# HIITMetagenomics/dsm-framework

Hardware: AMD Instinct MI355X
Metric: enumerated substrings/sec (Emax=2.0) (higher is better)
Workload: dtype u32

## Files before the change

dsm-framework_amd/csrc/engine.hip:

```cpp
#include <sched.h>

#include <algorithm>
#include <atomic>
#include <chrono>
#include <cmath>
#include <condition_variable>
#include <cstdlib>
#include <cstring>
#include <deque>
#include <map>
#include <functional>
#include <memory>
#include <mutex>
#include <sstream>
#include <thread>
#include <type_traits>

#include "common.h"
#include "scan.h"
#include "setorder.h"
#include "stream_parse.h"
#include "lfstep.h"
#include "entropy_tables.h"
#include "textemit.h"
#include "engine_api.h"
#include "emit_runs.h"

namespace dsm {

__device__ __forceinline__ u64 wave_sum_u64(u64 v) {
#pragma unroll
    for (int d = 32; d >= 1; d >>= 1) v += __shfl_xor(v, d, 64);
    return v;
}


struct Kids {
    const u64* plane;
    const u32* cum;
};
__device__ __forceinline__ u32 kid_mask(const Kids& k, u32 v) {
    const u64* p = k.plane + (size_t)(v >> 6) * 4;
    const u32 s = v & 63;
    return (u32)((p[0] >> s) & 1) | ((u32)((p[1] >> s) & 1) << 1) | ((u32)((p[2] >> s) & 1) << 2) | ((u32)((p[3] >> s) & 1) << 3);
}
__device__ __forceinline__ u32 kid_index(const Kids& k, u32 v, u32 c) {
    const size_t e = (size_t)(v >> 6) * 4 + c;
    return k.cum[e] + (u32)__popcll(k.plane[e] & ((1ull << (v & 63)) - 1));
}

struct KidWave {
    u64 p[4];
    u32 c[4];
};
__device__ __forceinline__ void kid_wave(const Kids& k, u32 w, KidWave& o) {
#pragma unroll
    for (int c = 0; c < 4; ++c) { o.p[c] = k.plane[(size_t)w * 4 + c]; o.c[c] = k.cum[(size_t)w * 4 + c]; }
}
__device__ __forceinline__ u32 bits_below_lane(u64 p) {
    return __builtin_amdgcn_mbcnt_hi((u32)(p >> 32), __builtin_amdgcn_mbcnt_lo((u32)p, 0u));
}

constexpr u32 NUM_XCD = 8;
__device__ __forceinline__ u32 xcd_block() {
    const u32 b = blockIdx.x, G = gridDim.x;
    const u32 x = b % NUM_XCD, i = b / NUM_XCD, per = G / NUM_XCD, rem = G % NUM_XCD;
    return x * per + (x < rem ? x : rem) + i;
}

constexpr int NPT = 4;
static inline dim3 grid_npt(u64 n) { return dim3((unsigned)((n + 256ull * NPT - 1) / (256ull * NPT))); }


static inline void timeline(const char* what, const char* arg = "") {
    static const bool on = getenv("DSM_TIMELINE") != nullptr;
    if (!on) return;
    static const auto t0 = std::chrono::steady_clock::now();
    fprintf(stderr, "dsm timeline %9.3f ms  %s %s\n", std::chrono::duration<double, std::milli>(std::chrono::steady_clock::now() - t0).count(), what, arg);
}

constexpr u32 BC_OK = 0x4f4b4f4bu, BC_CAPACITY = 0x46554c4cu, BC_ABORT = 0x41424f52u;
constexpr u32 XHDR = 16;
struct ExpandChain {
    struct Link { hipEvent_t last = nullptr; const void* owner = nullptr; };
    std::mutex mu;
    std::map<int, Link> dev;
};
static ExpandChain g_expand_chain;

struct Xchg {
    const u8* base;
    u64 bpr;
    u32 nlocal;
    u32 d;
    u64 F;
    u32 fb;
    u32 nm;
};
__device__ __forceinline__ u64 x_word_index(const Xchg& x, u32 l, u64 v) { return x.nm ? v * x.nlocal + l : (u64)l * x.F + v; }
__device__ __forceinline__ void x_split(const Xchg& x, u32 g, u32& r, u32& l) {
    if (x.nlocal == 1) { r = g; l = 0; }
    else if (x.d == x.nlocal) { r = 0; l = g; }
    else { r = g / x.nlocal; l = g % x.nlocal; }
}
template <typename P>
__device__ __forceinline__ P x_freq(const Xchg& x, u32 g, u64 v) {
    u32 r, l;
    x_split(x, g, r, l);
    const u8* rb = x.base + (u64)r * x.bpr + XHDR;
    if (x.fb == 1) return (P)(reinterpret_cast<const u16*>(rb)[x_word_index(x, l, v)] & (PACK_FMAX - 1));
    if (x.fb == 2) return (P)reinterpret_cast<const u16*>(rb)[(u64)l * x.F + v];
    return reinterpret_cast<const P*>(rb)[(u64)l * x.F + v];
}
template <typename P>
__device__ __forceinline__ u32 x_pl(const Xchg& x, u32 g, u64 v) {
    u32 r, l;
    x_split(x, g, r, l);
    if (x.fb == 1) return (u32)reinterpret_cast<const u16*>(x.base + (u64)r * x.bpr + XHDR)[x_word_index(x, l, v)] >> 9;
    const u8* rb = x.base + (u64)r * x.bpr + XHDR + (u64)x.nlocal * x.F * x.fb;
    return rb[(u64)l * x.F + v];
}

__device__ __forceinline__ bool x_is_nm8(const Xchg& x) { return x.nm && x.fb == 1 && x.nlocal == 8 && x.d == 8; }
__device__ __forceinline__ void x_words8(const Xchg& x, u64 v, u32 w[8]) {
    const uint4 q = reinterpret_cast<const uint4*>(x.base + XHDR)[v];
    w[0] = q.x & 0xFFFFu; w[1] = q.x >> 16; w[2] = q.y & 0xFFFFu; w[3] = q.y >> 16;
    w[4] = q.z & 0xFFFFu; w[5] = q.z >> 16; w[6] = q.w & 0xFFFFu; w[7] = q.w >> 16;
}

constexpr int MAX_LOCAL = 273;

template <typename P>
__device__ __forceinline__ void parent_eval(const Xchg& x, u32 u, u32 nT4[4]) {
    const u32 world = x.d / x.nlocal;
#pragma unroll
    for (int c = 0; c < 4; ++c) nT4[c] = 0;
    for (u32 r = 0; r < world; ++r) {
        if (x.fb == 1) {
            const u16* pw = reinterpret_cast<const u16*>(x.base + (u64)r * x.bpr + XHDR);
            if (x.nm && x.nlocal == 8) {
// ... 336 lines not shown
        cum[c] = base[c] + before;
    }
    u32 nT4[4] = {0, 0, 0, 0};
    if (o.sinfo) {
        if (in) { nT4[0] = sq.x & 0xFFFFu; nT4[1] = sq.x >> 16; nT4[2] = sq.y & 0xFFFFu; nT4[3] = sq.y >> 16; }
    } else {
#pragma unroll
        for (int c = 0; c < 4; ++c) nT4[c] = (u32)((up[c] >> lane) & 1);
    }
    if (lane < 4) {
        o.kcum[(size_t)w * 4 + lane] = DSM_PICK(cum, lane);
        if (o.kplane_w) o.kplane_w[(size_t)w * 4 + lane] = DSM_PICK(up, lane);
        if (o.cnt_clear && wi == 0) o.cnt_clear[(size_t)lane * o.nbp + tile] = 0;
    }
    if (o.cand_copy) {
        if (lane == 4) o.candbits[w] = candw;
        if (lane == 5) o.wsum[w] = candw;
    }
    u32 pres = 0, lastT = 0, vj[4];
#pragma unroll
    for (int c = 0; c < 4; ++c) {
        vj[c] = cum[c] + (u32)__popcll(up[c] & lt);
        if (nT4[c]) { pres |= 1u << c; lastT = nT4[c]; }
    }
    const u32 nc = __popc(pres);
    if (!in) myT = 0;
    const u32 same = o.single ? 1u : ((nc == 1 && lastT == myT) ? 1u : 0u);
    if (o.filter_on) {
        bool cand;
        if (o.single) {
            const FilterArgs& a = o.fa;
            cand = in && a.depth >= a.mindepth && 1u >= a.pmin && nc != 1 && !(f1 != 0 && l1 >= 1 && l1 <= 4);
            if (cand && a.emax > 0) {
                const u64 sumN = 1ull + f1;
                const double sl = f1 ? (double)(f1 + 1) * (double)__log2f((float)(f1 + 1)) : 0.0;
                const double e = (double)__log2f((float)sumN) - sl / (double)sumN;
                if (e < a.emin - ENT_MARGIN || e > a.emax + ENT_MARGIN) cand = false;
            }
        } else {
            cand = in && filter_node<P>(o.fa, x, u, myT, nc, same);
        }
        const u64 bits = __ballot(cand);
        u64 pairs = (u64)__popcll(bits);
        if (!o.single) pairs = wave_sum_u64(cand ? (u64)myT : 0ull);
        if (lane == 0) { o.candbits[w] = bits; o.wsum[w] = (u64)__popcll(bits) | (pairs << 32); }
    }
    if (!in) return;
    if (!o.single) o.samechild[u] = (u8)same;
#pragma unroll
    for (int c = 0; c < 4; ++c) {
        if (((pres >> c) & 1u) && vj[c] < o.cap) {
            if (o.slot) o.slot[vj[c]] = 4u * u + (u32)c;
            if (pw) pw[vj[c]] = child_path_word(mypw, u, o.plevel, (u32)c);
            if (o.sa) o.sa[vj[c]] = make_uint2(u, (u32)c | ((pres & ((1u << c) - 1u)) ? 0u : SREC_FIRST) | ((pres >> (c + 1)) ? 0u : SREC_LAST));
            if (!o.single) o.nT[vj[c]] = (u16)nT4[c];
        }
    }
    if (o.single) {
#pragma unroll
        for (int c = 0; c < 4; ++c)
            if (((pres >> c) & 1u) && vj[c] < o.cap) o.rp0[vj[c]] = (u32)c * o.seg + w * 64u + (u32)__popcll(up[c] & lt);
        return;
    }
    for (u32 sl = 0; sl < o.nlocal && pres && (o.tpos || o.rp_index); ++sl) {
        u32* rp = o.rp[sl];
        if (o.tpos) {
            const u32 m = x_pl<P>(x, o.rank * o.nlocal + sl, u) & 15u;
            const u32 h = m ? o.tpos[sl][u] : 0u;
#pragma unroll
            for (int c = 0; c < 4; ++c)
                if (((pres >> c) & 1u) && vj[c] < o.cap) rp[vj[c]] = ((m >> c) & 1u) ? h + (u32)__popc(m & ((1u << c) - 1u)) : DEAD;
        } else {
            const u64* sp = o.splane[sl] + (size_t)w * 4;
#pragma unroll
            for (int c = 0; c < 4; ++c) {
                if (!((pres >> c) & 1u) || vj[c] >= o.cap) continue;
                const u64 mine = sp[c];
                rp[vj[c]] = ((mine >> lane) & 1) ? (u32)c * o.seg + w * 64u + (u32)__popcll(mine & lt) : DEAD;
            }
        }
    }
}

template <typename P>
__global__ __launch_bounds__(256) void advance_single_kernel(Xchg x, AdvanceOut o) {
    const int lane = threadIdx.x & 63;
    const u32 F = (u32)x.F;
    const u32 nw = (F + 63) >> 6;
    const u32 tile = (u32)__builtin_amdgcn_readfirstlane((int)(xcd_block() * 4 + (threadIdx.x >> 6)));
    if (tile >= o.nbp) return;
    const u64 lt = (1ull << lane) - 1;
    const u64* __restrict__ line = o.kplane + (size_t)tile * 32;
    uint2 mypw[4];
#pragma unroll
    for (int q = 0; q < 4; ++q) {
        const u32 u = (tile * 4 + (u32)q) * 64 + lane;
        mypw[q] = o.parent_pw[u < F ? u : 0u];
    }
    u64 copyw = 0;
    if (lane < 32) copyw = line[lane];
    u32 cum[4];
#pragma unroll
    for (int c = 0; c < 4; ++c) cum[c] = o.cnt4[(size_t)c * o.nbp + tile];
    u64 up[4][4];
#pragma unroll
    for (int q = 0; q < 4; ++q)
#pragma unroll
        for (int c = 0; c < 4; ++c) up[q][c] = tile * 4 + (u32)q < nw ? line[q * 8 + c] : 0ull;
    {
        const u32 q = (u32)lane >> 3, j = (u32)lane & 7u, w = tile * 4 + q;
        if (lane < 32 && w < nw) {
            if (j < 4) o.kplane_w[(size_t)w * 4 + j] = copyw;
            else if (o.cand_copy && j == 4) o.candbits[w] = copyw;
            else if (o.cand_copy && j == 5) o.wsum[w] = copyw;
        }
    }
    const u32 r = o.plevel & (PW_CHUNK - 1);
    u32 kc = 0;
    u32 cbase = 0;
    u64 cbq[4] = {0, 0, 0, 0};
    u32 ncq[4] = {0, 0, 0, 0};
    u64 fq[4] = {0, 0, 0, 0};
    if (o.crec) {
        cbase = o.cnt4[(size_t)4 * o.nbp + tile] - o.cnt4[(size_t)4 * o.nbp];
#pragma unroll
        for (int q = 0; q < 4; ++q) {
            if (tile * 4 + (u32)q < nw) { cbq[q] = line[q * 8 + 4]; ncq[q] = (u32)line[q * 8 + 5]; }
            const u32 u = (tile * 4 + (u32)q) * 64 + lane;
            if ((cbq[q] >> lane) & 1ull) fq[q] = (u64)x_freq<P>(x, 0, u);
        }
    }
#pragma unroll
    for (int q = 0; q < 4; ++q) {
        const u32 w = tile * 4 + (u32)q, u = w * 64 + lane;
        const uint2 ppw = mypw[q];
        if (o.crec && cbq[q]) {
            const u32 k = cbase + bits_below_lane(cbq[q]);
            if (((cbq[q] >> lane) & 1ull) && k < o.crec_cap) o.crec[k] = make_uint4(u, 0u, (u32)fq[q], (u32)(fq[q] >> 32));
        }
        cbase += ncq[q];
#pragma unroll
        for (int c = 0; c < 4; ++c) {
            const u64 m = up[q][c];
            if (lane == q * 4 + c) kc = cum[c];
            const u32 below = bits_below_lane(m);
            const u32 vj = cum[c] + below;
            if (((m >> lane) & 1ull) && vj < o.cap) {
                o.rp0[vj] = (u32)c * o.seg + w * 64u + below;
                o.pw[vj] = r == 0 ? make_uint2(u, (u32)c) : make_uint2(ppw.x, ppw.y | ((u32)c << (2 * r)));
            }
            cum[c] += (u32)__popcll(m);
        }
    }
    if (lane < 16 && tile * 4 + ((u32)lane >> 2) < nw) o.kcum[(size_t)tile * 16 + lane] = kc;
}

__global__ __launch_bounds__(256) void lite_count_kernel(const u64* __restrict__ kplane, u32 nw, u32* __restrict__ cnt4, u32 nbp, u32 kshift, u32 cand_row = 0) {
    const u32 tile = blockIdx.x * 64 + (threadIdx.x >> 2), c = threadIdx.x & 3;
    if (tile >= nbp) return;
    u32 s = 0, nc = 0;
    if (cand_row && tile * 4 + c < nw) nc = (u32)kplane[((size_t)(tile * 4 + c) << 3) + 5];
#pragma unroll
    for (u32 q = 0; q < 4; ++q) {
        const u32 w = tile * 4 + q;
        if (w < nw) s += (u32)__popcll(kplane[((size_t)w << kshift) + c]);
    }
    cnt4[(size_t)c * nbp + tile] = s;
    if (cand_row) {
        nc += __shfl_xor(nc, 1, 64);
        nc += __shfl_xor(nc, 2, 64);
        if (c == 0) cnt4[(size_t)4 * nbp + tile] = nc;
    }
}
__global__ __launch_bounds__(256) void lite_slot_kernel(const u64* __restrict__ kplane, u32 F, const u32* __restrict__ cnt4, u32 nbp, u32 single_tile,
                                                        u32* __restrict__ slot, u32 cap) {
    const int lane = threadIdx.x & 63;
    const u32 nw = (F + 63) >> 6;
    const u32 tile = xcd_block();
    const u32 wi = threadIdx.x >> 6, w = tile * 4 + wi;
    if (w >= nw) return;
    const u32 u = w * 64 + lane;
    u32 base = 0;
#pragma unroll
    for (int c = 0; c < 4; ++c) {
        u32 before = 0, all = 0;
#pragma unroll
        for (u32 q = 0; q < 4; ++q) {
            const u32 wq = tile * 4 + q;
            const u32 t = wq < nw ? (u32)__popcll(kplane[(size_t)wq * 4 + c]) : 0u;
            before += q < wi ? t : 0u;
            all += t;
        }
        const u64 up = kplane[(size_t)w * 4 + c];
        const u32 first = (single_tile ? base : cnt4[(size_t)c * nbp + tile]) + before;
        base += all;
        const u32 vj = first + (u32)__popcll(up & ((1ull << lane) - 1));
        if (u < F && ((up >> lane) & 1) && vj < cap) slot[vj] = 4u * u + (u32)c;
    }
}

template <typename P>
__global__ __launch_bounds__(256) void order_kernel(u32 F, Xchg x, const u16* __restrict__ nT, const u64* __restrict__ order, Kids kids,
                                                    u64* __restrict__ order_next) {
    __shared__ u32 qn;
    __shared__ u32 qu[256];
    __shared__ u64 qm[256], qo[256];
    if (threadIdx.x == 0) qn = 0;
    __syncthreads();
    const u32 u = blockIdx.x * blockDim.x + threadIdx.x;
    if (u < F) {
        const u32 cnt = nT[u];
        const u64 ord = order[u];
        u64 mbyid = 0;
        u32 um = 0;
        if (x_is_nm8(x)) {
            u32 w[8];
            x_words8(x, u, w);
#pragma unroll
            for (int g = 0; g < 8; ++g) { const u32 m = (w[g] >> 9) & 15u; mbyid |= (u64)m << (4 * g); um |= m; }
        } else {
            for (u32 k = 0; k < cnt; ++k) {
                const u32 r = (u32)((ord >> (4 * k)) & 15);
                const u32 m = x_pl<P>(x, r, u) & 15u;
                mbyid |= (u64)m << (4 * r);
                um |= m;
            }
        }
        if (um && !(um & (um - 1))) {
            u64 rev = 0;
            for (u32 k = 0; k < cnt; ++k) {
                const u32 r = (u32)((ord >> (4 * k)) & 15);
                if ((mbyid >> (4 * r)) & 15) rev = (rev << 4) | r;
            }
            order_next[kid_index(kids, u, (u32)(__ffs((int)um) - 1))] = rev;
        } else if (um) {
            const u32 q = atomicAdd(&qn, 1u);
            qu[q] = u; qm[q] = mbyid; qo[q] = ord;
        }
    }
    __syncthreads();
    for (u32 q = threadIdx.x; q < qn; q += blockDim.x) {
        const u32 v = qu[q];
        const u64 mbyid = qm[q], ord = qo[q];
        const u32 cnt = nT[v];
        u64 ins[4] = {0, 0, 0, 0};
        u32 icnt[4] = {0, 0, 0, 0};
        for (u32 k = 0; k < cnt; ++k) {
            u32 r = (u32)((ord >> (4 * k)) & 15);
            u32 m = (u32)((mbyid >> (4 * r)) & 15);
// ... 96 lines not shown
                    l = l == 0xFF ? lg : (l == lg ? l : 5u);
                    sumN += f;
                    if (a.emax > 0) s += (double)(f + 1) * (double)__log2f((float)(f + 1));
                }
            }
            if (l >= 1 && l <= 4) out[i] = false;
            if (out[i] && a.emax > 0) {
                double e = (double)__log2f((float)sumN) - s / (double)sumN;
                if (e < a.emin - ENT_MARGIN || e > a.emax + ENT_MARGIN) out[i] = false;
            }
        }
        if (w < nw) {
            const u64 bits = __ballot(out[i]);
            u64 pairs = (u64)__popcll(bits);
            if (!one) pairs = wave_sum_u64(out[i] ? (u64)t[i] : 0ull);
            if (lane == 0) { candbits[w] = bits; wsum[w] = (u64)__popcll(bits) | (pairs << 32); }
        }
    }
}

template <typename P>
__global__ __launch_bounds__(256) void cand_store_kernel(FilterArgs a, Xchg x, const u16* __restrict__ nT, const u64* __restrict__ order,
                                                         const u16* __restrict__ order16, const u64* __restrict__ candbits,
                                                         const u64* __restrict__ wscan, u32* __restrict__ cand_node, u32* __restrict__ cand_poff,
                                                         u32* __restrict__ ids, u64* __restrict__ freqs) {
    const int lane = threadIdx.x & 63;
    const u32 nw = (a.F + 63) >> 6, stride = gridDim.x * 4;
    const u32 w0 = (u32)__builtin_amdgcn_readfirstlane((int)(xcd_block() * 4 + (threadIdx.x >> 6)));
    u64 bitsv[NPT], basev[NPT];
#pragma unroll
    for (int i = 0; i < NPT; ++i) {
        const u32 w = w0 + (u32)i * stride, wc = w < nw ? w : 0u;
        bitsv[i] = w < nw ? candbits[wc] : 0ull;
        basev[i] = wscan[wc];
    }
#pragma unroll
    for (int i = 0; i < NPT; ++i) {
        const u32 w = w0 + (u32)i * stride;
        const u64 bits = bitsv[i];
        if (!bits) continue;
        const u64 base = basev[i];
        const bool mine = (bits >> lane) & 1;
        const u32 v = w * 64 + lane;
        const u32 cnt = mine ? (a.d > 1 ? (u32)nT[v] : 1u) : 0u;
        const u32 k = (u32)(base & 0xFFFFFFFFu) + bits_below_lane(bits);
        u32 o = k;
        if (a.d > 1) o = (u32)(base >> 32) + (wave_inclusive_scan<u32>(cnt) - cnt);
        if (!mine) continue;
        cand_node[k] = v;
        cand_poff[k] = o;
        const u64 j = v;
        if (a.exact_order == 1) {
            const u64 ord = order[v];
            for (u32 q = 0; q < cnt; ++q) {
                u32 g = (u32)((ord >> (4 * q)) & 15);
                ids[o] = g; freqs[o] = (u64)x_freq<P>(x, g, j); ++o;
            }
        } else if (a.exact_order == 2) {
            const u16* ord = order16 + (size_t)v * a.d;
            for (u32 q = 0; q < cnt; ++q) {
                u32 g = ord[q];
                ids[o] = g; freqs[o] = (u64)x_freq<P>(x, g, j); ++o;
            }
        } else {
            for (u32 g = 0; g < a.d; ++g) {
                u64 f = (u64)x_freq<P>(x, g, j);
                if (f) { ids[o] = g; freqs[o] = f; ++o; }
            }
        }
    }
}

template <typename P>
__global__ void keep_kernel(u32 F, Xchg x, const uint2* __restrict__ sa, uint4* __restrict__ srec, u8* __restrict__ clen) {
    u32 v = blockIdx.x * blockDim.x + threadIdx.x;
    if (v >= F) return;
    const uint2 a = sa[v];
    const u64 f = (u64)x_freq<P>(x, 0, v);
    const u64 w = f | ((u64)(x_pl<P>(x, 0, v) >> 4) << 61);
    srec[v] = make_uint4(a.x, a.y, (u32)w, (u32)(w >> 32));
    clen[v] = (u8)((f < 128 ? 1u : 1u + (u32)((64 - __clzll((long long)f) + 7) >> 3)) + 2u);
}

template <typename T, typename OwnT>
__global__ __launch_bounds__(256) void up_kernel(u32 F, const OwnT* __restrict__ own, Kids kids, const T* __restrict__ child_agg,
                                                 T* __restrict__ agg) {
    const int lane = threadIdx.x & 63;
    const u32 nw = (F + 63) >> 6, stride = gridDim.x * 4;
    const u32 w0 = (u32)__builtin_amdgcn_readfirstlane((int)(xcd_block() * 4 + (threadIdx.x >> 6)));
    KidWave kw[NPT];
    T s[NPT];
#pragma unroll
    for (int i = 0; i < NPT; ++i) {
        const u32 w = w0 + (u32)i * stride, wc = w < nw ? w : 0u;
        const u32 v = wc * 64 + lane;
        s[i] = v < F ? (own ? (T)own[v] : (T)1) : (T)0;
        if (child_agg) kid_wave(kids, wc, kw[i]);
    }
    if (child_agg) {
        T g[NPT][4];
#pragma unroll
        for (int i = 0; i < NPT; ++i)
#pragma unroll
            for (int c = 0; c < 4; ++c) g[i][c] = child_agg[((kw[i].p[c] >> lane) & 1) ? kw[i].c[c] + bits_below_lane(kw[i].p[c]) : 0u];
#pragma unroll
        for (int i = 0; i < NPT; ++i)
#pragma unroll
            for (int c = 0; c < 4; ++c) s[i] += ((kw[i].p[c] >> lane) & 1) ? g[i][c] : (T)0;
    }
#pragma unroll
    for (int i = 0; i < NPT; ++i) {
        const u32 w = w0 + (u32)i * stride, v = w * 64 + lane;
        if (w < nw && v < F) agg[v] = s[i];
    }
}
template <typename T>
__global__ __launch_bounds__(256) void up_bits_kernel(u32 F, const u64* __restrict__ ownbits, Kids kids, const T* __restrict__ child_agg,
                                                      T* __restrict__ agg) {
    const int lane = threadIdx.x & 63;
    const u32 nw = (F + 63) >> 6, stride = gridDim.x * 4;
    const u32 w0 = (u32)__builtin_amdgcn_readfirstlane((int)(xcd_block() * 4 + (threadIdx.x >> 6)));
    KidWave kw[NPT];
    T s[NPT];
#pragma unroll
    for (int i = 0; i < NPT; ++i) {
        const u32 w = w0 + (u32)i * stride, wc = w < nw ? w : 0u;
        s[i] = ownbits ? (T)((ownbits[wc] >> lane) & 1) : (T)0;
        if (child_agg) kid_wave(kids, wc, kw[i]);
    }
    if (child_agg) {
        T g[NPT][4];
#pragma unroll
        for (int i = 0; i < NPT; ++i)
#pragma unroll
            for (int c = 0; c < 4; ++c) g[i][c] = child_agg[((kw[i].p[c] >> lane) & 1) ? kw[i].c[c] + bits_below_lane(kw[i].p[c]) : 0u];
#pragma unroll
        for (int i = 0; i < NPT; ++i)
#pragma unroll
            for (int c = 0; c < 4; ++c) s[i] += ((kw[i].p[c] >> lane) & 1) ? g[i][c] : (T)0;
    }
#pragma unroll
    for (int i = 0; i < NPT; ++i) {
        const u32 w = w0 + (u32)i * stride, v = w * 64 + lane;
        if (w < nw && v < F) agg[v] = s[i];
    }
}
template <typename T>
__global__ __launch_bounds__(256) void down_kernel(u32 F, const T* __restrict__ start, T lead, Kids kids,
                                                   const T* __restrict__ child_agg, T* __restrict__ child_start) {
    const int lane = threadIdx.x & 63;
    const u32 nw = (F + 63) >> 6, stride = gridDim.x * 4;
    const u32 w0 = (u32)__builtin_amdgcn_readfirstlane((int)(xcd_block() * 4 + (threadIdx.x >> 6)));
    KidWave kw[NPT];
    T s[NPT];
#pragma unroll
    for (int i = 0; i < NPT; ++i) {
        const u32 w = w0 + (u32)i * stride, wc = w < nw ? w : 0u;
        const u32 v = wc * 64 + lane;
        kid_wave(kids, wc, kw[i]);
        s[i] = start[v < F ? v : 0u] + lead;
    }
    T g[NPT][3];
#pragma unroll
    for (int i = 0; i < NPT; ++i)
#pragma unroll
        for (int c = 0; c < 3; ++c) {
            const bool need = ((kw[i].p[c] >> lane) & 1) && ((((kw[i].p[1] >> lane) & 1) << 1 | ((kw[i].p[2] >> lane) & 1) << 2 | ((kw[i].p[3] >> lane) & 1) << 3) >> (c + 1)) != 0;
            g[i][c] = child_agg[need ? kw[i].c[c] + bits_below_lane(kw[i].p[c]) : 0u];
        }
#pragma unroll
    for (int i = 0; i < NPT; ++i) {
        const u32 w = w0 + (u32)i * stride;
        if (w >= nw) continue;
        const u32 m = (u32)((kw[i].p[0] >> lane) & 1) | ((u32)((kw[i].p[1] >> lane) & 1) << 1) | ((u32)((kw[i].p[2] >> lane) & 1) << 2) |
                      ((u32)((kw[i].p[3] >> lane) & 1) << 3);
        T acc = s[i];
#pragma unroll
        for (int c = 0; c < 4; ++c) {
            if ((m >> c) & 1u) {
                child_start[kw[i].c[c] + bits_below_lane(kw[i].p[c])] = acc;
                if (c < 3 && (m >> (c + 1))) acc += g[i][c];
            }
        }
    }
}

struct RankSlot {
    u32 k, level;
    __device__ explicit operator u32() const { return level; }
};
__global__ void cand_rank_kernel(u32 ncand, const u32* __restrict__ cand_node, const u32* __restrict__ cand_poff, u32 npairs,
                                 const u32* __restrict__ start, const u32* __restrict__ sub, u32 level, RankSlot* __restrict__ slot,
                                 u32* __restrict__ npair, const uint4* __restrict__ crec) {
    u32 k = blockIdx.x * blockDim.x + threadIdx.x;
    if (k >= ncand) return;
    u32 v = crec ? crec[k].x : cand_node[k];
    u32 r = start[v] + sub[v] - 1;
    slot[r] = RankSlot{k, level};
    if (npair) npair[r] = crec ? 1u : (k + 1 < ncand ? cand_poff[k + 1] : npairs) - cand_poff[k];
}

struct LevelDev {
    const uint2* pw;
    const u32* cand_node;
    const u32* cand_poff;
    const uint4* crec;
    const u32* ids;
    const u64* freqs;
};

constexpr int EMIT_MAX_CHUNKS = 8;
struct ChunkBounds { u32 tb[EMIT_MAX_CHUNKS + 1]; int n; };
__global__ void chunk_bounds_kernel(ChunkBounds cbs, const u32* __restrict__ path_off, const u32* __restrict__ pair_off, u32* __restrict__ out) {
    const int c = threadIdx.x;
    if (c <= cbs.n) { out[2 * c] = path_off[cbs.tb[c]]; out[2 * c + 1] = pair_off ? pair_off[cbs.tb[c]] : cbs.tb[c]; }
}

constexpr u8 EV_DROP = 0, EV_KEEP = 1, EV_HOST = 2;
struct FillVerdict {
    double* ent;
    u8* keep;
    u32* rel_path;
    u32* rel_pair;
    u32* counts;
    const double* terms;
    const double* logn;
    const u32* bounds;
    u32 chunk, d;
// ... 1505 lines not shown
        const size_t need = wc * 12 + 512 + ((wc + TILE - 1) / TILE * 4) * 48 + 4096;
        if (arena.off + need <= arena.cap) return 0;
        const u32 hdr[4] = {BC_CAPACITY, 0, 0, 0};
        DSM_HIP(hipMemcpyAsync(bc_buf, hdr, 16, hipMemcpyHostToDevice, st));
        DSM_HIP(hipStreamSynchronize(st));
        w.owed.disarm();
        if (prm.bcast(prm.owner_ctx, owner, bc_buf, bc_bytes, (void*)st)) return fail(DSM_E_SINK, "bcast callback failed");
        return fail(DSM_E_CAPACITY, "device arena exhausted: use a longer prefix or a larger arena_bytes");
    }

    int advance(Walk& w, Sweep& s) {
        const u32 F = w.F, depth = w.depth;
        const int cur = w.cur(), nxt = cur ^ 1;
        s.x = xview(cur, F, w.w16, w.w9);
        const Xchg& x = s.x;
        LevelHost& me = w.L[depth];
        if (stream_mode && depth >= 1) {
            ARENA_GET(me.srec, uint4, F);
            ARENA_GET(me.clen, u8, F);
            hipLaunchKernelGGL((keep_kernel<P>), grid_for(F), dim3(256), 0, st, F, x, sa[cur], me.srec, me.clen);
        }
        if (!stream_mode && w.emitting && depth >= 1 && depth >= w.o.emit_lo && depth <= w.o.emit_hi) {
            int erc = emit_alloc(me, F);
            if (erc == DSM_E_CAPACITY && multi) { w.emit_failed = true; w.emitting = false; }
            else if (erc) return erc;
            else s.filtered = true;
        }
        s.mark = arena.off;
        const bool keep_slot = self_mode, keep_pw = !stream_mode;
        const size_t wcap = (size_t)F * 4 < Fcap ? (size_t)F * 4 : Fcap;
        u8* window = arena.get<u8>(wcap * ((keep_slot ? 4 : 0) + (keep_pw ? 8 : 0)) + 512);
        if (!window) return fail(DSM_E_CAPACITY, "device arena exhausted: use a longer prefix or a larger arena_bytes");
        s.slot = keep_slot ? reinterpret_cast<u32*>(window) : nullptr;
        const u32 nbp = (F + TILE - 1) / TILE;
        AdvanceOut ao;
        memset(&ao, 0, sizeof ao);
        ao.slot = s.slot; ao.nT = nT[nxt]; ao.samechild = samechild;
        if (stream_mode) ao.sa = sa[nxt];
        if (keep_pw) {
            ao.pw = reinterpret_cast<uint2*>(window);
            ao.pw_after_slot = keep_slot ? 1u : 0u;
            ao.parent_pw = me.pw;
            ao.plevel = depth;
        }
        ao.parent_nT = nT[cur]; ao.nlocal = (u32)nlocal; ao.rank = (u32)rank;
        ao.cap = (u32)wcap;
        ao.seg = seg_of(w.w16 && !trie_mode);
        ao.h_totals = d_pub_tot;
        ao.rp = d_rp_tab[nxt];
        ao.rp0 = rp[nxt][0];
        ao.tpos = trie_mode ? d_tpos_tab : nullptr;
        ao.splane = d_splane_tab;
        ao.rp_index = self_mode ? 0u : 1u;
        ao.kcum = me.kcum; ao.cnt4 = cnt4; ao.nbp = nbp; ao.kshift = 2;
        ao.width = d_totals;
        const bool merged = d > 1 || trie_mode;
        if (merged && nbp == 1) {
            ao.eval = 1; ao.kplane_w = me.kplane;
        } else if (merged) {
            hipLaunchKernelGGL((advance_reduce_kernel<P>), dim3(nbp), dim3(256), 0, st, x, sinfo, me.kplane, cnt4, nbp);
            ao.kplane = me.kplane; ao.sinfo = sinfo;
        } else {
            ao.kplane = splane[0]; ao.kplane_w = me.kplane; ao.single = 1;
            ao.kshift = 3;
        }
        const bool lean = !merged && nbp > 1 && keep_pw && !keep_slot && !stream_mode;
        if (lean && s.filtered && carena.cap) {
            const size_t room = (carena.cap - carena.off) / sizeof(uint4);
            s.crec_cap = (u32)(room < (size_t)F ? room : (size_t)F);
        }
        const bool fold = s.crec_cap > 0;
        if (nbp > 1) {
            if (!merged) hipLaunchKernelGGL(lite_count_kernel, dim3((nbp + 63) / 64), dim3(256), 0, st, splane[0], (F + 63) >> 6, cntraw, nbp, 3u, fold ? 1u : 0u);
            exclusive_scan<u32, u32>(merged ? cnt4 : cntraw, cnt4, (size_t)(fold ? 5 : 4) * nbp, scan_tmp, d_totals, st);
        }
        const bool fused_filter = s.filtered && nbp > 1;
        if (fused_filter) {
            ao.fa = filter_args(F, depth, w.order_mode); ao.candbits = me.cand_bits; ao.wsum = cand_wsum;
            if (ao.single) ao.cand_copy = 1;
            else ao.filter_on = 1;
        }
        if (fold) { ao.crec = reinterpret_cast<uint4*>(carena.base + carena.off); ao.crec_cap = s.crec_cap; }
        if (nbp == 1) hipLaunchKernelGGL((advance_down_kernel<P>), dim3(1), dim3(256), 0, st, x, ao);
        else if (lean) hipLaunchKernelGGL((advance_single_kernel<P>), dim3((nbp + 3) / 4), dim3(256), 0, st, x, ao);
        else hipLaunchKernelGGL((advance_wave_kernel<P>), dim3(nbp), dim3(256), 0, st, x, ao);
        if (s.filtered) {
            if (int erc = emit_filter(me, F, depth, x, cur, w.order_mode, !fused_filter, fold)) return erc;
        }
        return 0;
    }

    int publish(Walk& w, Sweep& s) {
        const u32 F = w.F, nbp = (F + TILE - 1) / TILE;
        const int nxt = w.cur() ^ 1;
        PublishArgs pa;
        memset(&pa, 0, sizeof pa);
        pa.total = nbp == 1 ? d_pub_tot : d_totals;
        pa.cmax_base = s.x.base; pa.cmax_bpr = s.x.bpr; pa.cmax_world = (u32)world;
        if (s.filtered) pa.cand = d_totals64;
        if (s.crec_cap) {
            pa.total = cnt4 + (size_t)4 * nbp;
            pa.grand = d_totals;
            pa.cand = nullptr;
        }
        pa.clear = reinterpret_cast<u32*>(multi ? xsend : xrecv[nxt]);
        pa.packet = reinterpret_cast<uint4*>(h_totals + 304); pa.seq = ++pub_seq;
        pa.next = spec_mode ? d_dyn : nullptr;
        pa.bc_header = owner_mode ? reinterpret_cast<uint4*>(bc_buf) : nullptr;
        hipLaunchKernelGGL(publish_kernel, dim3(1), dim3(64), 0, st, pa);
        if (owner_mode) {
            const size_t bc_bytes = bcast_bytes(F);
            DSM_HIP(hipMemcpyAsync(bc_buf + 16, w.L[w.depth].kplane, bc_bytes - 16, hipMemcpyDeviceToDevice, st));
            w.owed.disarm();
            if (prm.bcast(prm.owner_ctx, owner, bc_buf, bc_bytes, (void*)st)) return fail(DSM_E_SINK, "bcast callback failed");
            stats.exchange_bytes_sent += bc_bytes * (u64)(world - 1);
        }
        if (spec_mode) { if (int rc = launch_lf(w, w.depth + 1, 0, w.w16, w.w9, s.slot, (u64)F * 4)) return rc; }
        u32 pk[4];
        if (int rc = wait_packet(pk)) return rc;
        s.Fn = decode_level(pk[1], &s.w16, &s.w9);
        s.spec_hit = spec_mode && s.Fn > 0 && s.Fn <= level_cap(s.w16) && s.w16 == w.w16 && s.w9 == w.w9;
        if (spec_mode && !s.spec_hit) --stats.expand_launches;
        h_totals[300] = pk[2]; h_totals[301] = pk[3];
        if (int rc = check_width(s.Fn, s.w16)) return rc;
        if (owner_mode) {
            if (!s.Fn) w.owed.arm(16);
            else w.owed.arm_next((size_t)level_bytes(s.Fn, s.w16, s.w9), xrecv[nxt], bcast_bytes(s.Fn));
        }
        return 0;
    }
    int wait_packet(u32 pk[4]) {
        volatile u32* fl = h_totals + 304;
        u32 spins = 0;
        while (*fl != pub_seq) {
            if ((++spins & 0xFFFFu) == 0 && hipStreamQuery(st) != hipErrorNotReady) {
                DSM_HIP(hipStreamSynchronize(st));
                if (*fl != pub_seq) return fail(DSM_E_HIP, "publish kernel did not report");
                break;
            }
            __builtin_ia32_pause();
        }
        std::atomic_thread_fence(std::memory_order_acquire);
        for (int q = 0; q < 4; ++q) pk[q] = fl[q];
        return 0;
    }

    int commit(Walk& w, const Sweep& s, LevelHost& child) {
        const u32 F = w.F, Fn = s.Fn;
        const int cur = w.cur(), nxt = cur ^ 1;
        arena.off = s.mark;
        child.n = Fn;
        if (!Fn) return 0;
        if (self_mode) child.slot = arena.get<u32>(Fn);
        if (!stream_mode) child.pw = arena.get<uint2>(Fn);
        if (int rc = alloc_kids(child)) return rc;
        if (s.spec_hit) {
            stats.expand_slots += Fn;
            stats.expand_column_bytes += (u64)Fn * col_bytes(s.w16, s.w9);
        } else {
            if (int rc = launch_lf(w, w.depth + 1, Fn, s.w16, s.w9, child.slot)) return rc;
        }
        const Kids kids = w.L[w.depth].kids();
        if (!(w.o.emit || w.o.capture)) {}
        else if (w.order_mode == 1)
            hipLaunchKernelGGL((order_kernel<P>), grid_for(F), dim3(256), 0, st, F, s.x, nT[cur], order[cur], kids, order[nxt]);
        else if (w.order_mode == 2 && d <= 64)
            hipLaunchKernelGGL((order_big_kernel<P, 64>), grid_for(F, 64), dim3(64), 0, st, F, s.x, nT[cur], order16[cur], kids, order16[nxt]);
// ... 120 lines not shown
                for (int c = 0; c < NCOUNTERS; ++c) hc[c] += sh[(size_t)k * 8 + c];
#ifdef DSM_CLOCK_PROBE
            if (sh[7]) {
                double dur = 0, ramp = 0, tail = 0, meanbusy = 0;
                int nl = 0;
                const double W = (double)lfgeo.blocks * lfgeo.waves_per_block;
                for (int k = 1; k + 2 < COUNTER_SHARDS; k += 3) {
                    const u64 s0 = ~sh[(size_t)k * 8 + 6], s9 = sh[(size_t)k * 8 + 7], e0 = ~sh[(size_t)(k + 1) * 8 + 6], e9 = sh[(size_t)(k + 1) * 8 + 7];
                    if (!s9 || e9 - s0 < 5000) continue;
                    const double ms = (double)sh[(size_t)(k + 2) * 8 + 6] / W, me = (double)sh[(size_t)(k + 2) * 8 + 7] / W;
                    dur += (double)(e9 - s0); ramp += (double)(s9 - s0); tail += (double)(e9 - e0); meanbusy += me - ms; ++nl;
                }
                fprintf(stderr, "clock probe: %.1f MHz; %d launches >= 50 us: duration %.2f ms, first-to-last wave start %.2f ms, first-to-last wave end %.2f ms, mean wave busy %.2f ms\n",
                        (double)sh[6] / (double)sh[7] * 100.0, nl, dur * 1e-5, ramp * 1e-5, tail * 1e-5, meanbusy * 1e-5);
            }
#endif
        }
        stats.reported += hc[0];
        stats.lf_steps += hc[1];
        stats.rank_ops += hc[2];
        stats.index_lines += hc[3];
        stats.record_bytes += hc[4];
        stats.records_read += hc[5];
        return 0;
    }

    FilterArgs filter_args(u32 F, u32 depth, u32 order_mode) const {
        FilterArgs fa;
        fa.F = F; fa.depth = depth; fa.d = d; fa.pmin = prm.pmin; fa.pmax = prm.pmax; fa.mindepth = prm.mindepth;
        fa.emin = prm.emin; fa.emax = prm.emax; fa.exact_order = order_mode;
        return fa;
    }
    int emit_alloc(LevelHost& me, u32 F) {
        EARENA_GET(me.cand_bits, u64, ((size_t)F + 63) / 64);
        return 0;
    }
    int emit_filter(LevelHost& me, u32 F, u32 depth, const Xchg& xp, int cur, u32 order_mode, bool run_kernel, bool stored = false) {
        const FilterArgs fa = filter_args(F, depth, order_mode);
        if (run_kernel)
            hipLaunchKernelGGL((filter_kernel<P>), grid_npt(F), dim3(256), 0, st, fa, xp, nT[cur], me.kids(), samechild, me.cand_bits, cand_wsum);
        if (!stored) exclusive_scan<u64, u64>(cand_wsum, cand_wscan, ((size_t)F + 63) / 64, scan_tmp64, d_totals64, st);
        return 0;
    }
    int emit_store(LevelHost& me, u32 F, u32 depth, const Xchg& xp, int cur, u32 order_mode, u32 stored_cap = 0) {
        const FilterArgs fa = filter_args(F, depth, order_mode);
        u64 tot = 0;
        memcpy(&tot, h_totals + 300, sizeof tot);
        me.ncand = (u32)(tot & 0xFFFFFFFFu);
        me.npairs = (u32)(tot >> 32);
        if (stored_cap && me.ncand <= stored_cap) {
            if (me.ncand) {
                me.crec = carena.get<uint4>(me.ncand);
                if (!me.crec) return fail(DSM_E_HIP, "candidate arena: the block that held the records cannot be claimed");
            }
            stats.candidates += me.ncand;
            return 0;
        }
        if (stored_cap)
            exclusive_scan<u64, u64>(cand_wsum, cand_wscan, ((size_t)F + 63) / 64, scan_tmp64, d_totals64, st);
        if (me.ncand) {
            u32 nc = me.ncand;
            me.ncand = 0;
            EARENA_GET(me.cand_node, u32, nc);
            EARENA_GET(me.cand_poff, u32, nc);
            EARENA_GET(me.ids, u32, me.npairs);
            EARENA_GET(me.freqs, u64, me.npairs);
            me.ncand = nc;
            hipLaunchKernelGGL((cand_store_kernel<P>), grid_npt(F), dim3(256), 0, st, fa, xp, nT[cur], order[cur], order16[cur], me.cand_bits, cand_wscan,
                               me.cand_node, me.cand_poff, me.ids, me.freqs);
        }
        stats.candidates += me.ncand;
        return 0;
    }

    int finish_mine(std::vector<LevelHost>& L, u32 nlev, dsm_tuple_sink sink, void* ctx, bool* ready) {
        u64 ncand_total = 0;
        for (u32 l = 1; l < nlev; ++l) ncand_total += L[l].ncand;
        if (ncand_total == 0) return 0;
        if (ncand_total > 0xFFFFFFF0ull) return fail(DSM_E_CAPACITY, "more than 2^32 candidate tuples in one prefix: use a longer prefix");
        const u32 nt = (u32)ncand_total;
        for (u32 l = nlev; l-- > 1;) {
            EARENA_GET(L[l].sub, u32, L[l].n);
            const u32* child_sub = l + 1 < nlev ? L[l + 1].sub : nullptr;
            hipLaunchKernelGGL((up_bits_kernel<u32>), grid_npt(L[l].n), dim3(256), 0, st, L[l].n, L[l].cand_bits, L[l].kids(), child_sub, L[l].sub);
        }
        const bool text_mode = text_sink_ != nullptr;
        const bool one_pair = d == 1 && !text_mode;
        u32* npair = nullptr;
        if (!one_pair) EARENA_GET(npair, u32, nt);
        u32 maxn = 1;
        for (u32 l = 0; l < nlev; ++l) maxn = L[l].n > maxn ? L[l].n : maxn;
        u32* startbuf[2];
        EARENA_GET(startbuf[0], u32, maxn);
        EARENA_GET(startbuf[1], u32, maxn);
        RankSlot* slot;
        EARENA_GET(slot, RankSlot, nt);
        DSM_HIP(hipMemsetAsync(startbuf[0], 0, sizeof(u32), st));
        for (u32 l = 0; l + 1 < nlev; ++l) {
            u32* s_cur = startbuf[l & 1];
            u32* s_next = startbuf[(l + 1) & 1];
            hipLaunchKernelGGL((down_kernel<u32>), grid_npt(L[l].n), dim3(256), 0, st, L[l].n, s_cur, 0u, L[l].kids(), L[l + 1].sub, s_next);
            if (L[l + 1].ncand)
                hipLaunchKernelGGL(cand_rank_kernel, grid_for(L[l + 1].ncand), dim3(256), 0, st, L[l + 1].ncand, L[l + 1].cand_node, L[l + 1].cand_poff,
                                   L[l + 1].npairs, s_next, L[l + 1].sub, l + 1, slot, npair, L[l + 1].crec);
        }
        std::vector<LevelDev> lv(nlev);
        u64 path_bytes = 0, npairs = 0;
        for (u32 l = 0; l < nlev; ++l) {
            lv[l].pw = L[l].pw; lv[l].cand_node = L[l].cand_node; lv[l].cand_poff = L[l].cand_poff; lv[l].crec = L[l].crec;
            lv[l].ids = L[l].ids; lv[l].freqs = L[l].freqs;
            if (l && L[l].ncand) { path_bytes += (u64)l * L[l].ncand; npairs += L[l].crec ? L[l].ncand : L[l].npairs; }
        }
        if (path_bytes > 0xFFFFFFFFull || npairs > 0xFFFFFFFFull) return fail(DSM_E_CAPACITY, "more than 2^32 path bytes or pairs in one prefix: use a longer prefix");
        LevelDev* d_lv;
        EARENA_GET(d_lv, LevelDev, nlev);
        DSM_HIP(hipMemcpyAsync(d_lv, lv.data(), nlev * sizeof(LevelDev), hipMemcpyHostToDevice, st));
        EmitSet& E = emitter.acquire();
        E.device = device;
        if (!E.ready) DSM_HIP(hipEventCreateWithFlags(&E.ready, hipEventDisableTiming));
        if (!copy_stream) DSM_HIP(hipStreamCreateWithFlags(&copy_stream, hipStreamNonBlocking));
        if (int rc = E.dev[0].ensure(((size_t)nt + 1) * 4)) return rc;
        if (!one_pair) { if (int rc = E.dev[1].ensure(((size_t)nt + 1) * 4)) return rc; }
        u32* path_off = (u32*)E.dev[0].p;
        u32* pair_off = one_pair ? nullptr : (u32*)E.dev[1].p;
        u32* stmp;
        EARENA_GET(stmp, u32, scan_tmp_elems(nt) + 8);
        exclusive_scan<RankSlot, u32>(slot, path_off, nt, stmp, d_totals, st);
        if (!one_pair) exclusive_scan<u32, u32>(npair, pair_off, nt, stmp, d_totals + 1, st);
        DSM_HIP(hipMemcpyAsync(path_off + nt, d_totals, sizeof(u32), hipMemcpyDeviceToDevice, st));
        if (!one_pair) DSM_HIP(hipMemcpyAsync(pair_off + nt, d_totals + 1, sizeof(u32), hipMemcpyDeviceToDevice, st));
        static const u64 chunk_unit = [] {
            const char* e = getenv("DSM_EMIT_CHUNK_TUPLES");
            const long long n = e ? atoll(e) : 0;
            return n > 0 ? (u64)n : (u64)(1u << 20);
        }();
        ChunkBounds cbs;
        cbs.n = nt >= 4 * chunk_unit ? 4 : (nt >= 2 * chunk_unit ? 2 : 1);
        for (int c = 0; c <= cbs.n; ++c) cbs.tb[c] = (u32)((u64)nt * c / cbs.n);
        u32* d_bounds;
        EARENA_GET(d_bounds, u32, 2 * (EmitSet::MAX_CHUNKS + 1));
        hipLaunchKernelGGL(chunk_bounds_kernel, dim3(1), dim3(64), 0, st, cbs, path_off, pair_off, d_bounds);
        DSM_HIP(hipMemcpyAsync(h_bounds, d_bounds, 2 * (cbs.n + 1) * sizeof(u32), hipMemcpyDeviceToHost, st));
        const bool no_ids = d == 1;
        if (!no_ids) { if (int rc = E.dev[2].ensure((size_t)npairs * 4)) return rc; }
        if (int rc = E.dev[3].ensure((size_t)npairs * 8)) return rc;
        if (int rc = E.dev[4].ensure((size_t)path_bytes)) return rc;
        u32* d_ids = no_ids ? nullptr : (u32*)E.dev[2].p;
        u64* d_freqs = (u64*)E.dev[3].p;
        char* d_paths = (char*)E.dev[4].p;
        emitter.text_sink = text_sink_;
        FillVerdict fv;
        memset(&fv, 0, sizeof fv);
        if (!text_mode) {
            const size_t nrel = (size_t)nt + EmitSet::MAX_CHUNKS + 1;
            if (int rc = E.pin[0].ensure(nrel * 4)) return rc;
            if (int rc = E.pin[1].ensure(nrel * 4)) return rc;
            if (!no_ids) { if (int rc = E.pin[2].ensure((size_t)npairs * 4)) return rc; }
            if (int rc = E.pin[3].ensure((size_t)npairs * 8)) return rc;
            if (int rc = E.pin[4].ensure((size_t)path_bytes)) return rc;
            if (int rc = E.pin[5].ensure((size_t)nt * 8)) return rc;
            if (int rc = E.pin[6].ensure((size_t)nt)) return rc;
            if (int rc = E.pin[9].ensure(2 * EmitSet::MAX_CHUNKS * sizeof(u32))) return rc;
            if (int rc = E.dev[5].ensure((size_t)nt * 8)) return rc;
            if (int rc = E.dev[6].ensure((size_t)nt)) return rc;
            if (int rc = E.dev[7].ensure(nrel * 4)) return rc;
            if (int rc = E.dev[8].ensure(nrel * 4)) return rc;
            if (int rc = E.dev[9].ensure(2 * EmitSet::MAX_CHUNKS * sizeof(u32))) return rc;
// ... 427 lines not shown
```

Baseline: 3.695 billion.

## Specialize advance/up kernels and restructure loads into wave-wide reads with readlane

advance_single_kernel now loads the tile's cnt4 counters and kplane line once per wave into vector registers and broadcasts them with readlane. It is templated on the frequency byte width so the frequency read becomes a direct typed load, and it uses empty asm hints to keep uniform values in scalar registers. up_bits_kernel and up_kernel are specialized at compile time on whether own bits and children exist, removing runtime branches. lite_count_kernel issues all of its loads up front without predication. The goal is fewer scalar/vector memory round trips and less divergent control flow, at the cost of more template instantiations and reliance on inline asm register-class hints.

```diff
diff --git a/dsm-framework_amd/csrc/engine.hip b/dsm-framework_amd/csrc/engine.hip
--- a/dsm-framework_amd/csrc/engine.hip
+++ b/dsm-framework_amd/csrc/engine.hip
@@ -49,6 +49,11 @@
     return k.cum[e] + (u32)__popcll(k.plane[e] & ((1ull << (v & 63)) - 1));
 }
 
+template <typename T>
+__device__ __forceinline__ void scalar_here(const T& v) { asm volatile("" ::"s"(v)); }
+template <typename T>
+__device__ __forceinline__ void vector_here(const T& v) { asm volatile("" ::"v"(v)); }
+
 struct KidWave {
     u64 p[4];
     u32 c[4];
@@ -56,6 +61,10 @@
 __device__ __forceinline__ void kid_wave(const Kids& k, u32 w, KidWave& o) {
 #pragma unroll
     for (int c = 0; c < 4; ++c) { o.p[c] = k.plane[(size_t)w * 4 + c]; o.c[c] = k.cum[(size_t)w * 4 + c]; }
+}
+__device__ __forceinline__ void kid_wave_here(const KidWave& o) {
+#pragma unroll
+    for (int c = 0; c < 4; ++c) { scalar_here(o.p[c]); scalar_here(o.c[c]); }
 }
 __device__ __forceinline__ u32 bits_below_lane(u64 p) {
     return __builtin_amdgcn_mbcnt_hi((u32)(p >> 32), __builtin_amdgcn_mbcnt_lo((u32)p, 0u));
@@ -558,33 +567,62 @@
     }
 }
 
-template <typename P>
+__device__ __forceinline__ u64 lane_word(u64 v, int L) {
+    const u32 lo = (u32)__builtin_amdgcn_readlane((int)(u32)v, L), hi = (u32)__builtin_amdgcn_readlane((int)(u32)(v >> 32), L);
+    return (u64)lo | ((u64)hi << 32);
+}
+template <typename P, int FB>
+__device__ __forceinline__ u64 single_freq(const Xchg& x, u32 v) {
+    const u8* col = x.base + XHDR;
+    if (FB == 1) return (u64)(reinterpret_cast<const u16*>(col)[v] & (PACK_FMAX - 1));
+    if (FB == 2) return (u64)reinterpret_cast<const u16*>(col)[v];
+    return (u64)reinterpret_cast<const P*>(col)[v];
+}
+template <typename P, int FB>
 __global__ __launch_bounds__(256) void advance_single_kernel(Xchg x, AdvanceOut o) {
     const int lane = threadIdx.x & 63;
     const u32 F = (u32)x.F;
     const u32 nw = (F + 63) >> 6;
     const u32 tile = (u32)__builtin_amdgcn_readfirstlane((int)(xcd_block() * 4 + (threadIdx.x >> 6)));
     if (tile >= o.nbp) return;
-    const u64 lt = (1ull << lane) - 1;
+    scalar_here(x.base); scalar_here(o.cnt4); scalar_here(o.kplane); scalar_here(o.kplane_w); scalar_here(o.candbits); scalar_here(o.wsum); scalar_here(o.cand_copy); scalar_here(o.crec);
+    scalar_here(o.crec_cap); scalar_here(o.cap); scalar_here(o.rp0); scalar_here(o.pw); scalar_here(o.seg); scalar_here(o.plevel); scalar_here(o.kcum);
     const u64* __restrict__ line = o.kplane + (size_t)tile * 32;
+    const bool rec = o.crec != nullptr;
     uint2 mypw[4];
+    u64 fq[4];
+#pragma unroll
+    for (int q = 0; q < 4; ++q) {
+        const u32 u = (tile * 4 + (u32)q) * 64 + lane, uc = u < F ? u : 0u;
+        mypw[q] = o.parent_pw[uc];
+    }
+    const u32 crow4 = rec ? 4u : 0u;
+    const u32 cl = (u32)lane & 7u;
+    const u32 cntw = o.cnt4[(size_t)(cl < 4 ? cl : crow4) * o.nbp + (cl < 4 || (cl == 4 && rec) ? tile : 0u)];
+    const u64 copyw = line[lane & 31];
+    vector_here(cntw); vector_here(copyw);
+    u32 cum[4];
+#pragma unroll
+    for (int c = 0; c < 4; ++c) cum[c] = (u32)__builtin_amdgcn_readlane((int)cntw, c);
+    u32 cbase = (u32)__builtin_amdgcn_readlane((int)cntw, 4) - (u32)__builtin_amdgcn_readlane((int)cntw, 5);
+    u64 up[4][4], cbq[4];
+    u32 ncq[4];
+#pragma unroll
+    for (int q = 0; q < 4; ++q) {
+        const u64 live = tile * 4 + (u32)q < nw ? ~0ull : 0ull;
+        const u64 liverec = rec ? live : 0ull;
+#pragma unroll
+        for (int c = 0; c < 4; ++c) up[q][c] = lane_word(copyw, q * 8 + c) & live;
+        cbq[q] = lane_word(copyw, q * 8 + 4) & liverec;
+        ncq[q] = (u32)__builtin_amdgcn_readlane((int)(u32)copyw, q * 8 + 5) & (u32)liverec;
+    }
 #pragma unroll
     for (int q = 0; q < 4; ++q) {
         const u32 u = (tile * 4 + (u32)q) * 64 + lane;
-        mypw[q] = o.parent_pw[u < F ? u : 0u];
-    }
-    u64 copyw = 0;
-    if (lane < 32) copyw = line[lane];
-    u32 cum[4];
-#pragma unroll
-    for (int c = 0; c < 4; ++c) cum[c] = o.cnt4[(size_t)c * o.nbp + tile];
-    u64 up[4][4];
-#pragma unroll
-    for (int q = 0; q < 4; ++q)
-#pragma unroll
-        for (int c = 0; c < 4; ++c) up[q][c] = tile * 4 + (u32)q < nw ? line[q * 8 + c] : 0ull;
+        fq[q] = single_freq<P, FB>(x, ((cbq[q] >> lane) & 1ull) ? u : 0u);
+    }
     {
-        const u32 q = (u32)lane >> 3, j = (u32)lane & 7u, w = tile * 4 + q;
+        const u32 q = ((u32)lane >> 3) & 3u, j = (u32)lane & 7u, w = tile * 4 + q;
         if (lane < 32 && w < nw) {
             if (j < 4) o.kplane_w[(size_t)w * 4 + j] = copyw;
             else if (o.cand_copy && j == 4) o.candbits[w] = copyw;
@@ -593,24 +631,11 @@
     }
     const u32 r = o.plevel & (PW_CHUNK - 1);
     u32 kc = 0;
-    u32 cbase = 0;
-    u64 cbq[4] = {0, 0, 0, 0};
-    u32 ncq[4] = {0, 0, 0, 0};
-    u64 fq[4] = {0, 0, 0, 0};
-    if (o.crec) {
-        cbase = o.cnt4[(size_t)4 * o.nbp + tile] - o.cnt4[(size_t)4 * o.nbp];
-#pragma unroll
-        for (int q = 0; q < 4; ++q) {
-            if (tile * 4 + (u32)q < nw) { cbq[q] = line[q * 8 + 4]; ncq[q] = (u32)line[q * 8 + 5]; }
-            const u32 u = (tile * 4 + (u32)q) * 64 + lane;
-            if ((cbq[q] >> lane) & 1ull) fq[q] = (u64)x_freq<P>(x, 0, u);
-        }
-    }
 #pragma unroll
     for (int q = 0; q < 4; ++q) {
         const u32 w = tile * 4 + (u32)q, u = w * 64 + lane;
         const uint2 ppw = mypw[q];
-        if (o.crec && cbq[q]) {
+        if (cbq[q]) {
             const u32 k = cbase + bits_below_lane(cbq[q]);
             if (((cbq[q] >> lane) & 1ull) && k < o.crec_cap) o.crec[k] = make_uint4(u, 0u, (u32)fq[q], (u32)(fq[q] >> 32));
         }
@@ -634,13 +659,21 @@
 __global__ __launch_bounds__(256) void lite_count_kernel(const u64* __restrict__ kplane, u32 nw, u32* __restrict__ cnt4, u32 nbp, u32 kshift, u32 cand_row = 0) {
     const u32 tile = blockIdx.x * 64 + (threadIdx.x >> 2), c = threadIdx.x & 3;
     if (tile >= nbp) return;
-    u32 s = 0, nc = 0;
-    if (cand_row && tile * 4 + c < nw) nc = (u32)kplane[((size_t)(tile * 4 + c) << 3) + 5];
+    u64 pw[4];
 #pragma unroll
     for (u32 q = 0; q < 4; ++q) {
         const u32 w = tile * 4 + q;
-        if (w < nw) s += (u32)__popcll(kplane[((size_t)w << kshift) + c]);
-    }
+        pw[q] = kplane[((size_t)(w < nw ? w : 0u) << kshift) + c];
+    }
+    const u32 wn = tile * 4 + c;
+    const bool hasn = cand_row && wn < nw;
+    const u64 nword = kplane[hasn ? ((size_t)wn << 3) + 5 : ((size_t)(tile * 4) << kshift) + c];
+#pragma unroll
+    for (u32 q = 0; q < 4; ++q) vector_here(pw[q]);
+    vector_here(nword);
+    u32 s = 0, nc = hasn ? (u32)nword : 0u;
+#pragma unroll
+    for (u32 q = 0; q < 4; ++q) s += tile * 4 + q < nw ? (u32)__popcll(pw[q]) : 0u;
     cnt4[(size_t)c * nbp + tile] = s;
     if (cand_row) {
         nc += __shfl_xor(nc, 1, 64);
@@ -903,7 +936,7 @@
     clen[v] = (u8)((f < 128 ? 1u : 1u + (u32)((64 - __clzll((long long)f) + 7) >> 3)) + 2u);
 }
 
-template <typename T, typename OwnT>
+template <typename T, typename OwnT, bool OWN, bool KIDS>
 __global__ __launch_bounds__(256) void up_kernel(u32 F, const OwnT* __restrict__ own, Kids kids, const T* __restrict__ child_agg,
                                                  T* __restrict__ agg) {
     const int lane = threadIdx.x & 63;
@@ -915,10 +948,14 @@
     for (int i = 0; i < NPT; ++i) {
         const u32 w = w0 + (u32)i * stride, wc = w < nw ? w : 0u;
         const u32 v = wc * 64 + lane;
-        s[i] = v < F ? (own ? (T)own[v] : (T)1) : (T)0;
-        if (child_agg) kid_wave(kids, wc, kw[i]);
-    }
-    if (child_agg) {
+        if (KIDS) kid_wave(kids, wc, kw[i]);
+        s[i] = OWN ? (T)own[v < F ? v : 0u] : (T)1;
+    }
+    if (KIDS) {
+#pragma unroll
+        for (int i = 0; i < NPT; ++i) kid_wave_here(kw[i]);
+    }
+    if (KIDS) {
         T g[NPT][4];
 #pragma unroll
         for (int i = 0; i < NPT; ++i)
@@ -935,21 +972,29 @@
         if (w < nw && v < F) agg[v] = s[i];
     }
 }
-template <typename T>
+template <typename T, bool OWN, bool KIDS>
 __global__ __launch_bounds__(256) void up_bits_kernel(u32 F, const u64* __restrict__ ownbits, Kids kids, const T* __restrict__ child_agg,
                                                       T* __restrict__ agg) {
     const int lane = threadIdx.x & 63;
     const u32 nw = (F + 63) >> 6, stride = gridDim.x * 4;
     const u32 w0 = (u32)__builtin_amdgcn_readfirstlane((int)(xcd_block() * 4 + (threadIdx.x >> 6)));
     KidWave kw[NPT];
-    T s[NPT];
+    u64 ob[NPT];
 #pragma unroll
     for (int i = 0; i < NPT; ++i) {
         const u32 w = w0 + (u32)i * stride, wc = w < nw ? w : 0u;
-        s[i] = ownbits ? (T)((ownbits[wc] >> lane) & 1) : (T)0;
-        if (child_agg) kid_wave(kids, wc, kw[i]);
-    }
-    if (child_agg) {
+        ob[i] = OWN ? ownbits[wc] : 0ull;
+        if (KIDS) kid_wave(kids, wc, kw[i]);
+    }
+#pragma unroll
+    for (int i = 0; i < NPT; ++i) {
+        if (OWN) scalar_here(ob[i]);
+        if (KIDS) kid_wave_here(kw[i]);
+    }
+    T s[NPT];
+#pragma unroll
+    for (int i = 0; i < NPT; ++i) s[i] = (T)((ob[i] >> lane) & 1);
+    if (KIDS) {
         T g[NPT][4];
 #pragma unroll
         for (int i = 0; i < NPT; ++i)
@@ -965,6 +1010,14 @@
         const u32 w = w0 + (u32)i * stride, v = w * 64 + lane;
         if (w < nw && v < F) agg[v] = s[i];
     }
+}
+template <typename T>
+static void launch_up_bits(hipStream_t st, u32 F, const u64* ownbits, Kids kids, const T* child_agg, T* agg) {
+    const dim3 grid = grid_npt(F), block(256);
+    if (ownbits && child_agg) hipLaunchKernelGGL((up_bits_kernel<T, true, true>), grid, block, 0, st, F, ownbits, kids, child_agg, agg);
+    else if (ownbits) hipLaunchKernelGGL((up_bits_kernel<T, true, false>), grid, block, 0, st, F, ownbits, kids, child_agg, agg);
+    else if (child_agg) hipLaunchKernelGGL((up_bits_kernel<T, false, true>), grid, block, 0, st, F, ownbits, kids, child_agg, agg);
+    else hipLaunchKernelGGL((up_bits_kernel<T, false, false>), grid, block, 0, st, F, ownbits, kids, child_agg, agg);
 }
 template <typename T>
 __global__ __launch_bounds__(256) void down_kernel(u32 F, const T* __restrict__ start, T lead, Kids kids,
@@ -2636,7 +2689,12 @@
         }
         if (fold) { ao.crec = reinterpret_cast<uint4*>(carena.base + carena.off); ao.crec_cap = s.crec_cap; }
         if (nbp == 1) hipLaunchKernelGGL((advance_down_kernel<P>), dim3(1), dim3(256), 0, st, x, ao);
-        else if (lean) hipLaunchKernelGGL((advance_single_kernel<P>), dim3((nbp + 3) / 4), dim3(256), 0, st, x, ao);
+        else if (lean) {
+            const dim3 grid((nbp + 3) / 4);
+            if (x.fb == 1) hipLaunchKernelGGL((advance_single_kernel<P, 1>), grid, dim3(256), 0, st, x, ao);
+            else if (x.fb == 2) hipLaunchKernelGGL((advance_single_kernel<P, 2>), grid, dim3(256), 0, st, x, ao);
+            else hipLaunchKernelGGL((advance_single_kernel<P, 0>), grid, dim3(256), 0, st, x, ao);
+        }
         else hipLaunchKernelGGL((advance_wave_kernel<P>), dim3(nbp), dim3(256), 0, st, x, ao);
         if (s.filtered) {
             if (int erc = emit_filter(me, F, depth, x, cur, w.order_mode, !fused_filter, fold)) return erc;
@@ -2923,7 +2981,7 @@
         for (u32 l = nlev; l-- > 1;) {
             EARENA_GET(L[l].sub, u32, L[l].n);
             const u32* child_sub = l + 1 < nlev ? L[l + 1].sub : nullptr;
-            hipLaunchKernelGGL((up_bits_kernel<u32>), grid_npt(L[l].n), dim3(256), 0, st, L[l].n, L[l].cand_bits, L[l].kids(), child_sub, L[l].sub);
+            launch_up_bits<u32>(st, L[l].n, L[l].cand_bits, L[l].kids(), child_sub, L[l].sub);
         }
         const bool text_mode = text_sink_ != nullptr;
         const bool one_pair = d == 1 && !text_mode;
```

Result: no change. 3.686 billion (-0.3%).
